# patrickzbhe/ray-tracing-series-rust

Measured on AMD Instinct MI355X. Metric: Msamples/s (pixels x spp) on Book-1 final scene, higher is better.
Workload: dtype f64

## Files before the change

ray-tracing-series-rust_amd/csrc/core/integrator.hpp:

```cpp
#pragma once
#include "shading.hpp"

namespace rt {

struct PathState {
  Ray ray;
  Color product;
  Color output;
  int32_t depth;
  Rng rng;
};

RT_HD void path_begin(const RenderParams& rp, uint32_t i, uint32_t j, uint32_t sample, PathState* ps) {
  uint64_t pixel_index = (uint64_t)j * (uint64_t)rp.image_width + (uint64_t)i;
  ps->rng = rng_for_sample(rp.seed, pixel_index, sample);
  real ru = rng_f64(ps->rng);
  real u = ((real)i + ru) / (real)(rp.image_width - 1);
  real rv = rng_f64(ps->rng);
  real v = ((real)j + rv) / (real)(rp.image_height - 1);
  ps->ray = camera_get_ray(rp.cam, u, v, ps->rng);
  ps->product = v3(1, 1, 1);
  ps->output = v3(0, 0, 0);
  ps->depth = rp.max_depth;
}

RT_HD bool path_bounce_begin(PathState* ps) {
  ps->depth -= 1;
#if defined(RT_F32)
  const real mag = rt_fabs(ps->ray.origin.x) + rt_fabs(ps->ray.origin.y) + rt_fabs(ps->ray.origin.z) +
                   rt_fabs(ps->ray.direction.x) + rt_fabs(ps->ray.direction.y) + rt_fabs(ps->ray.direction.z);
  if (!(mag < RT_INFINITY)) return true;
#endif
  return ps->depth < 0;
}

template <uint32_t F, bool COUNT>
RT_HD bool path_bounce_end(const SceneView& sv, const RenderParams& rp, PathState* ps, bool hit,
                           const HitRecord& rec, TraceCounters* cnt) {
  if (!hit) {
    ps->output += ps->product * rp.background;
    return true;
  }
  const FlatMaterial& m = sv.materials[rec.mat];
  Ray scattered;
  Color attenuation;
  bool did_scatter = material_scatter<F, COUNT>(sv, m, ps->ray, rec, ps->rng, &scattered, &attenuation, cnt);
  Color emitted = material_emitted<F, COUNT>(sv, m, rec, cnt);
  ps->output += emitted * ps->product;
  if (!did_scatter) return true;
  ps->product *= attenuation;
  ps->ray = scattered;
  return false;
}

enum LightKind : int32_t { LIGHT_RECT = 0, LIGHT_SPHERE = 1 };
struct FlatLight {
  int32_t kind;
  int32_t slot;
  int32_t prim;
  int32_t mat;
  real area;
  real cdf;
  real pmf;
};
struct LightView {
  const FlatLight* lights;
  const int32_t* slot_light;
  int32_t n_lights;
  int32_t pad;
};

#define RT_NEE_SHADOW_EPS real(1e-6)

RT_HD real mis_power(real a, real b) {
  const real a2 = a * a, b2 = b * b;
  return a2 / (a2 + b2);
}

RT_HD real light_pdf_rect(const FlatRect& q, real area, Vec3 d) {
  const real dn = rt_fabs(q.axis == RECT_XY ? d.z : (q.axis == RECT_XZ ? d.y : d.x));
  const real d2 = length_squared(d);
  return d2 * rt_sqrt(d2) / (dn * area);
}
RT_HD real sphere_cone_one_minus(const FlatSphere& s, Point3 p) {
  const Vec3 oc = v3(s.cx, s.cy, s.cz) - p;
  const real d2 = length_squared(oc), r2 = s.radius * s.radius;
  if (!(d2 > r2)) return real(0.0);
  const real k = r2 / d2;
  return k / (real(1.0) + rt_sqrt(real(1.0) - k));
}
RT_HD real light_pdf_sphere(const FlatSphere& s, Point3 p) {
  const real om = sphere_cone_one_minus(s, p);
  return om > real(0.0) ? real(1.0) / (real(2.0) * RT_PI * om) : real(0.0);
}
RT_HD real light_pdf(const SceneView& sv, const LightView& lv, int32_t k, Point3 p, Point3 q) {
  const FlatLight& L = lv.lights[k];
  const real ps = L.kind == LIGHT_RECT ? light_pdf_rect(sv.rects[L.prim], L.area, q - p) : light_pdf_sphere(sv.spheres[L.prim], p);
  return L.pmf * ps;
}

RT_HD real nee_bsdf_pdf(int32_t kind, const HitRecord& rec, Vec3 dir) {
  if (kind == MAT_ISOTROPIC) return real(1.0) / (real(4.0) * RT_PI);
  const real c = dot(rec.normal, dir) / length(dir);
  return c > real(0.0) ? c / RT_PI : real(0.0);
}

template <uint32_t F, bool COUNT, class STACK>
RT_HD Color nee_connect(const SceneView& sv, const LightView& lv, const PathState* ps, const HitRecord& rec, int32_t kind,
                        Color albedo, Rng& rng, STACK& stack, TraceCounters* cnt) {
  const real ul = rng_f64(rng);
  int32_t k = 0;
  while (k + 1 < lv.n_lights && !(ul < lv.lights[k].cdf)) ++k;
  const FlatLight& L = lv.lights[k];
  const real u1 = rng_f64(rng), u2 = rng_f64(rng);
  const Point3 p = rec.p;
  Point3 q;
  real pdf_sa;
  HitRecord lrec;
  lrec.u = real(0.0); lrec.v = real(0.0);
  if (L.kind == LIGHT_RECT) {
    const FlatRect& r = sv.rects[L.prim];
    const real a = r.a0 + u1 * (r.a1 - r.a0), b = r.b0 + u2 * (r.b1 - r.b0);
    q = r.axis == RECT_XY ? v3(a, b, r.k) : (r.axis == RECT_XZ ? v3(a, r.k, b) : v3(r.k, a, b));
    if (F & F_IMAGE) {
      lrec.u = (a - r.a0) / (r.a1 - r.a0);
      lrec.v = (b - r.b0) / (r.b1 - r.b0);
    }
    pdf_sa = light_pdf_rect(r, L.area, q - p);
  } else {
    const FlatSphere& s = sv.spheres[L.prim];
    const Point3 c = v3(s.cx, s.cy, s.cz);
    const real om = sphere_cone_one_minus(s, p);
    if (!(om > real(0.0))) return v3(0, 0, 0);
    const Vec3 w = unit(c - p);
    const Vec3 a = rt_fabs(w.x) > real(0.9) ? v3(0, 1, 0) : v3(1, 0, 0);
// ... 113 lines not shown
```

ray-tracing-series-rust_amd/csrc/hip/render.hip:

```cpp
#include <hip/hip_runtime.h>
#include <cstdio>
#include <cstdlib>
#include <algorithm>
#include <chrono>
#include <cfloat>
#include <cmath>
#include <cstring>
#include <new>
#include <type_traits>
#include <utility>
#include <string>
#include <vector>
#include "../../../include/rtx_abi.h"
#include "../core/cull32.hpp"
#include "../core/integrator.hpp"
#include "../host/flat_scene.hpp"
#include "../host/light_table.hpp"
#include "device_buffer.hpp"
#include "f32_bridge.hpp"
#ifndef RTX_F32_TU
#include "abi_internal.hpp"
#else
namespace rtx { void set_error(const std::string& msg); }
#endif

namespace rtx {

#include "pass_items.inc"

struct FlatNode4;
typedef const FlatNode4 FlatNode4Dev;
struct WorldDesc;

struct LdsSceneDims {
  uint32_t n_nodes, n_refs, n_spheres, n_moving;
  uint32_t node_dwords;
  uint32_t n_uni;
};

struct VoteTop {
  int32_t n;
  int32_t all_rects;
  int32_t k[8];
  uint32_t ref[8];
  rt::FlatRect rect[8];
};

enum class ForcedKernel { none, simple, vote, world, wavefront };

struct TraceSwitches {
  ForcedKernel kernel = ForcedKernel::none;
  bool diag = false;
  int ring = -1, wide = -1, scene_lds = -1;
  bool vote_top = true, tri_direct = true, mat_lds = true, perlin_lds = true;
  bool mv_common = true, motion = true, motion_axis = true;
  bool single_leaf = true, pass_pipeline = true, validate = false;
  uint32_t chunk = TRACE_CHUNK;
  uint32_t world_threshold = 8;
  uint32_t walk_threshold = 0, regen_min = 0, leaf_weight = 0;
  uint32_t wf_paths = 1u << 22, wf_refill = 16, wf_check = 8;
  int wf_occ = 4;
  bool wf_verbose = false;
};

struct Workspace {
  DeviceBuffer<double> samples;
  DeviceBuffer<double> accum;
  DeviceBuffer<rt::TraceCounters> counters;
  DeviceBuffer<unsigned int> work_counter;
  DeviceBuffer<unsigned long long> diag;
  hipEvent_t ev[2] = {nullptr, nullptr};
  hipStream_t aux_stream = nullptr;
  hipEvent_t ev_pass[3] = {nullptr, nullptr, nullptr};
  DeviceBuffer<unsigned char> wave_mem;
  uint32_t* wave_host_ctrl = nullptr;
};

struct VotePlan {
  bool ok = false;
  int32_t bvh_pos = 0;
  int32_t tri_base = -1;
  VoteTop top;
  int blocks_per_cu[2] = {1, 1};
  bool ring[2] = {false, false};
  uint32_t tables = 0;
  size_t tables_bytes = 0;
};

struct WidePlan {
  FlatNode4Dev* nodes4 = nullptr;
  int levels = 0;
  int vote_blocks_per_cu = 1;
};

struct WorldPlan {
  const WorldDesc* desc = nullptr;
  uint32_t mat_lds = 0, tex_lds = 0;
  uint32_t perlin_lds = 0;
  int blocks_per_cu[5][2] = {{1, 1}, {1, 1}, {1, 1}, {1, 1}, {1, 1}};
};

struct LdsFit {
  bool ok = false;
  uint32_t ring_cap = 0;
  uint32_t levels = 0;
  LdsSceneDims dims = {0, 0, 0, 0, 0, 0};
};

struct LdsPlan {
  LdsFit plain;
  LdsFit motion;
  int motion_axis = -1;
  double motion_t0 = 0.0, motion_t1 = 0.0;
  bool mv_common = false;
  double mv_t0 = 0.0, mv_t1 = 1.0;
};

struct WalkTuning {
  uint32_t walk_threshold = 18;
  uint32_t regen_min = 1;
  uint32_t leaf_weight = 3;
  bool single_leaf = false;
};

struct DeviceScene {
  int device = -1;
  std::vector<DeviceBuffer<void>> allocations;
  rt::SceneView view;
  size_t scene_bytes = 0;
  int n_cu = 256;
  double gravity_time_limit = 1e300;
  TraceSwitches sw;
  Workspace ws;
  VotePlan vote;
  WidePlan wide;
  WorldPlan world;
  LdsPlan lds;
  WalkTuning walk;
  rt::LightView lights = {nullptr, nullptr, 0, 0};
};

#define HIP_TRY(expr)                                                                      \
  do {                                                                                     \
    hipError_t _e = (expr);                                                                \
    if (_e != hipSuccess) {                                                                \
      set_error(std::string(#expr) + ": " + hipGetErrorString(_e));                        \
      return RTX_EHIP;                                                                     \
    }                                                                                      \
  } while (0)

template <class T>
static rtx_status upload_array(DeviceScene* ds, const std::vector<T>& v, const T** out) {
  *out = nullptr;
  if (v.empty()) return RTX_OK;
  DeviceBuffer<void> b;
  size_t bytes = v.size() * sizeof(T);
  HIP_TRY(b.alloc(bytes));
  HIP_TRY(hipMemcpy(b, v.data(), bytes, hipMemcpyHostToDevice));
  ds->scene_bytes += bytes;
  *out = (const T*)(void*)b;
  ds->allocations.push_back(std::move(b));
  return RTX_OK;
}

static void free_device_scene(DeviceScene* ds) {
  if (!ds) return;
  Workspace& ws = ds->ws;
  if (ws.wave_host_ctrl) (void)hipHostFree(ws.wave_host_ctrl);
  for (int i = 0; i < 2; ++i)
    if (ws.ev[i]) (void)hipEventDestroy(ws.ev[i]);
  for (int i = 0; i < 3; ++i)
    if (ws.ev_pass[i]) (void)hipEventDestroy(ws.ev_pass[i]);
  if (ws.aux_stream) (void)hipStreamDestroy(ws.aux_stream);
  delete ds;
}

template <class T>
__device__ __forceinline__ T dev_load_uniform(const T* p) { return *(const __attribute__((address_space(4))) T*)(p); }

__device__ __forceinline__ unsigned long long wave_ballot(bool p) { return __builtin_amdgcn_ballot_w64(p); }

#define TRACE_BLOCK 256
struct LdsStack {
  int32_t* base;
  int n;
  static constexpr bool kBottom = false;
  __device__ __forceinline__ void reset() { n = 0; }
  __device__ __forceinline__ void push(int32_t v) { base[n * TRACE_BLOCK] = v; ++n; }
  __device__ __forceinline__ int32_t pop() { --n; return base[n * TRACE_BLOCK]; }
  __device__ __forceinline__ bool empty() const { return n == 0; }
};
struct LdsStackB {
  int32_t* base;
  int n;
  static constexpr bool kBottom = true;
  __device__ __forceinline__ void reset() { base[0] = 0x7fffffff; n = 1; }
  __device__ __forceinline__ void init() { reset(); }
  __device__ __forceinline__ void push(int32_t v) { base[n * TRACE_BLOCK] = v; ++n; }
  __device__ __forceinline__ int32_t pop() { --n; return base[n * TRACE_BLOCK]; }
  __device__ __forceinline__ int32_t top() const { return base[(n - 1) * TRACE_BLOCK]; }
  __device__ __forceinline__ bool empty() const { return n <= 1; }
};

__device__ __forceinline__ void flush_counters(const rt::TraceCounters& c, rt::TraceCounters* g) {
  atomicAdd(&g->box_tests, c.box_tests);
  atomicAdd(&g->sphere_tests, c.sphere_tests);
  atomicAdd(&g->moving_sphere_tests, c.moving_sphere_tests);
  atomicAdd(&g->rect_tests, c.rect_tests);
  atomicAdd(&g->triangle_tests, c.triangle_tests);
  atomicAdd(&g->scatters, c.scatters);
  atomicAdd(&g->texels, c.texels);
  atomicAdd(&g->perlin_calls, c.perlin_calls);
  atomicAdd(&g->rays, c.rays);
  atomicAdd(&g->samples, c.samples);
}

#define DIAG_ADD(region, mask) do { if (DIAG) { dg[2 * (region)] += 1; dg[2 * (region) + 1] += (unsigned long long)__popcll(mask); } } while (0)
#include "trace_basic.inc"
#include "trace_vote.inc"
#include "trace_world.inc"
#include "trace_lds.inc"
#include "trace_wave.inc"
#include "post_kernels.inc"
#include "denoise.inc"
#ifndef RTX_F32_TU
#include "trace_nee.inc"
#endif

static int shard_row_count(int32_t height, const RtxShard& sh, int32_t row_limit) {
  int n = 0;
  for (int32_t j = 0; j < height && j < row_limit; ++j)
    if ((j / sh.block_rows) % sh.shard_count == sh.shard_index) ++n;
  return n;
}

static rtx_status validate(const void* s, const RtxCamera* cam, const RtxConfig* cfg,
                           const RtxShard* shard, RtxShard* sh_out) {
  if (!s || !cam || !cfg) { set_error("render: NULL scene, camera or config"); return RTX_EINVAL; }
  if (cfg->threads <= 0 || cfg->image_width <= 0 || cfg->samples_per_pixel <= 0 || cfg->max_depth <= 0) {
    set_error("render: Config::new asserts threads, image_width, samples_per_pixel, max_depth > 0 (world.rs:36-40)");
    return RTX_EINVAL;
  }
  if (rtx_image_height(cfg) <= 0) { set_error("render: image height <= 0 (Screen::new asserts, screen.rs:14)"); return RTX_EINVAL; }
  if (!(cam->time1 < cam->time2)) { set_error("render: camera time1 >= time2 (gen_range panics on an empty range, camera.rs:69)"); return RTX_EINVAL; }
  RtxShard sh = {0, 1, 1, 0};
  if (shard) sh = *shard;
  if (sh.shard_count <= 0 || sh.shard_index < 0 || sh.shard_index >= sh.shard_count || sh.block_rows <= 0) {
    set_error("render: bad shard");
    return RTX_EINVAL;
  }
  *sh_out = sh;
  return RTX_OK;
}

static rt::RenderParams make_params(const RtxCamera* cam, const RtxConfig* cfg) {
  rt::RenderParams rp;
  static_assert(sizeof(RtxCamera) == 24 * sizeof(double) && sizeof(rt::FlatCamera) == 24 * sizeof(rt::real), "camera layout");
  for (int k = 0; k < 24; ++k) ((rt::real*)&rp.cam)[k] = (rt::real)((const double*)cam)[k];
  rp.background = rt::v3(cfg->background[0], cfg->background[1], cfg->background[2]);
  rp.image_width = cfg->image_width;
  rp.image_height = rtx_image_height(cfg);
  rp.samples_per_pixel = cfg->samples_per_pixel;
  rp.max_depth = cfg->max_depth;
  rp.seed = cfg->seed;
  return rp;
}

static TraceSwitches read_switches() {
  auto num = [](const char* n, int lo, int hi, uint32_t dflt) { const char* s = getenv(n); return s && atoi(s) >= lo && atoi(s) <= hi ? (uint32_t)atoi(s) : dflt; };
  auto flag = [](const char* n) { const char* s = getenv(n); return s ? (atoi(s) != 0 ? 1 : 0) : -1; };
  TraceSwitches sw;
  if (const char* k = getenv("RTX_TRACE_KERNEL")) {
    const std::string s = k;
    if (s == "simple") sw.kernel = ForcedKernel::simple;
    else if (s == "vote" || s == "vote_diag") sw.kernel = ForcedKernel::vote;
    else if (s == "world" || s == "world_diag") sw.kernel = ForcedKernel::world;
    else if (s == "wavefront") sw.kernel = ForcedKernel::wavefront;
    sw.diag = s == "vote_diag" || s == "world_diag";
  }
  sw.ring = flag("RTX_RING"); sw.wide = flag("RTX_WIDE"); sw.scene_lds = flag("RTX_SCENE_LDS");
  sw.vote_top = flag("RTX_VOTE_TOP") != 0; sw.tri_direct = flag("RTX_TRI_DIRECT") != 0;
  sw.mat_lds = flag("RTX_MAT_LDS") != 0; sw.perlin_lds = flag("RTX_PERLIN_LDS") != 0;
  sw.mv_common = flag("RTX_MV_COMMON") != 0; sw.motion = flag("RTX_MOTION") != 0; sw.motion_axis = flag("RTX_MOTION_AXIS") != 0;
  sw.single_leaf = flag("RTX_SINGLE_LEAF") != 0; sw.pass_pipeline = flag("RTX_PASS_PIPELINE") != 0;
  sw.validate = getenv("RTX_VALIDATE") != nullptr;
  sw.chunk = num("RTX_CHUNK", 64, 65536, sw.chunk);
  sw.world_threshold = num("RTX_WORLD_THRESHOLD", 0, 64, sw.world_threshold);
  sw.walk_threshold = num("RTX_WALK_THRESHOLD", 1, 64, 0); sw.regen_min = num("RTX_REGEN_MIN", 1, 64, 0); sw.leaf_weight = num("RTX_LEAF_WEIGHT", 1, 64, 0);
  const char* wp = getenv("RTX_WF_PATHS");
  if (wp && atol(wp) >= 256 && atol(wp) <= (1l << 27)) sw.wf_paths = (uint32_t)atol(wp);
  sw.wf_refill = num("RTX_WF_REFILL", 1, 64, sw.wf_refill); sw.wf_check = num("RTX_WF_CHECK", 1, 4096, sw.wf_check);
  sw.wf_occ = (int)num("RTX_WF_OCC", 4, 6, (uint32_t)sw.wf_occ); sw.wf_verbose = getenv("RTX_WF_VERBOSE") != nullptr;
  return sw;
}

static size_t stack_bytes(uint32_t levels) { return (size_t)levels * TRACE_BLOCK * sizeof(int32_t); }

template <class K>
static int occupancy(K kernel, size_t lds) {
  int nb = 0;
  return hipOccupancyMaxActiveBlocksPerMultiprocessor(&nb, kernel, TRACE_BLOCK, lds) == hipSuccess ? nb : 0;
}

static uint32_t grid_size(uint32_t total, uint32_t block, uint64_t resident) {
  const uint64_t want = ((uint64_t)total + block - 1) / block;
  return (uint32_t)(want < resident ? want : resident);
}

struct PassArgs {
  rt::RenderParams rp;
  ShardMap sm;
  uint32_t s_begin, total, npix;
  double* samples;
  unsigned int* work_counter;
  hipStream_t stream;
  int preset;
  uint32_t feat;
  uint32_t stack_levels;
  size_t stack_lds;
  const uint32_t* active;
};

template <class Launch>
static void with_map(const PassArgs& a, Launch launch) {
  if (a.active) launch(ActiveMap{a.sm, a.active});
  else launch(a.sm);
}

template <class Launch>
static rtx_status run_diag(DeviceScene* ds, hipStream_t stream, Launch launch, const char* tag, int width, const char* const* names,
                           int n, unsigned long long (&h)[24]) {
  if (!ds->ws.diag) HIP_TRY(ds->ws.diag.alloc(sizeof(h)));
  HIP_TRY(hipMemsetAsync(ds->ws.diag, 0, sizeof(h), stream));
  launch();
  HIP_TRY(hipStreamSynchronize(stream));
  HIP_TRY(hipMemcpy(h, ds->ws.diag, sizeof(h), hipMemcpyDeviceToHost));
  for (int k = 0; k < n; ++k)
    fprintf(stderr, "[%s] %-*s executions %llu lanes %llu mean lanes %.2f\n", tag, width, names[k], h[2 * k], h[2 * k + 1],
            h[2 * k] ? (double)h[2 * k + 1] / (double)h[2 * k] : 0.0);
  return RTX_OK;
}

struct LeafScan { uint32_t max_count = 0, max_end = 0; };
static LeafScan scan_leaves(const FlatScene& fs) {
  LeafScan s;
  for (const rt::FlatNode& nd : fs.nodes)
    for (int ch = 0; ch < 2; ++ch)
      if (nd.child[ch] < 0) {
        s.max_count = std::max(s.max_count, rt::leaf_count(nd.child[ch]));
        s.max_end = std::max(s.max_end, rt::leaf_first(nd.child[ch]) + rt::leaf_count(nd.child[ch]));
      }
  return s;
}

static void plan_vote(DeviceScene* ds, const FlatScene& fs) {
  VotePlan& p = ds->vote;
  const TraceSwitches& sw = ds->sw;
  const size_t lds = stack_bytes((uint32_t)fs.max_stack + 1u), lds_ring = lds + (TRACE_BLOCK / 64) * ring_bytes(64);
  const bool ring_fits = lds_ring <= 64 * 1024;
  auto fit = [&](int preset, int nb0, int nb1, bool ring_by_default) {
    p.ring[preset] = ring_by_default && nb1 > 0 && nb1 >= nb0 && ring_fits;
    if (sw.ring >= 0 && nb1 > 0 && ring_fits) p.ring[preset] = sw.ring != 0;
    const int nb = p.ring[preset] ? nb1 : nb0;
    if (nb > 0) p.blocks_per_cu[preset] = nb;
  };
  fit(0, occupancy(k_trace_vote<P_SPHERES, false, false, false>, lds), occupancy(k_trace_vote<P_SPHERES, false, true, false>, lds_ring), true);
  fit(1, occupancy(k_trace_vote<P_MESH, false, false, false>, lds), occupancy(k_trace_vote<P_MESH, false, true, false>, lds_ring), false);

  memset(&p.top, 0, sizeof(p.top));
  p.top.n = -1;
  int n_bvh = 0, n_other = 0;
// ... 228 lines not shown

static void fit_lds(LdsFit* f, bool want_ring, uint32_t lds_max) {
  for (uint32_t cap : {64u, 48u, 0u})
    if ((want_ring || cap == 0u) && ldsk_layout(f->levels, cap, f->dims).total <= lds_max) {
      f->ok = true;
      f->ring_cap = cap;
      return;
    }
}

static rtx_status plan_lds(DeviceScene* ds, const FlatScene& fs, const LeafScan& leaves) {
  const bool single_bvh = fs.top_level.size() == 1 && fs.entries[fs.top_level[0]].kind == rt::ENTRY_BVH;
  if (!single_bvh || (fs.features & ~P_SPHERES) != 0 || fs.nodes32.size() > LDSK_MAX_NODES) return RTX_OK;
  LdsPlan& p = ds->lds;
  const TraceSwitches& sw = ds->sw;
  const uint32_t max_end = leaves.max_end, levels = (uint32_t)fs.max_stack + 1u;
  int lds_max = 0;
  (void)hipDeviceGetAttribute(&lds_max, hipDeviceAttributeMaxSharedMemoryPerBlock, ds->device);
  if (lds_max > 160 * 1024) lds_max = 160 * 1024;
  p.plain.levels = levels;
  p.plain.dims = {(uint32_t)fs.nodes32.size(), max_end, max_end, 0u, LDSK_NODE_DWORDS, 0u};
  if (!fs.moving_spheres.empty()) {
    bool same = sw.mv_common;
    for (const rt::FlatMovingSphere& ms : fs.moving_spheres)
      same = same && ms.time0 == fs.moving_spheres[0].time0 && ms.time1 == fs.moving_spheres[0].time1;
    if (same) { p.mv_common = true; p.mv_t0 = (double)fs.moving_spheres[0].time0; p.mv_t1 = (double)fs.moving_spheres[0].time1; }
  }
  if (fs.features & rt::F_MOVING_SPHERE) {
    p.plain.dims.n_uni = (uint32_t)fs.spheres.size();
    p.plain.dims.n_moving = max_end;
    p.plain.dims.n_spheres = 0u;
  }
  p.motion.levels = levels;
  p.motion.dims = p.plain.dims;
  p.motion.dims.node_dwords = LDSK_MOTION_NODE_DWORDS;
  {
    bool moves[3] = {false, false, false};
    for (const rt::FlatMotion32& m : fs.motion32)
      for (int ch = 0; ch < 2; ++ch)
        for (int a = 0; a < 3; ++a) moves[a] = moves[a] || m.dlo[ch][a] != 0.0f || m.dhi[ch][a] != 0.0f;
    if (!fs.motion32.empty() && moves[1] && !moves[0] && !moves[2] && sw.motion_axis) {
      p.motion_axis = 1;
      p.motion.dims.node_dwords = LDSK_MOTION1_NODE_DWORDS;
    }
  }
  if (leaves.max_count <= 4 && max_end <= LDSK_MAX_SLOTS && sw.scene_lds != 0 && lds_max > 0) {
    const bool want_ring = sw.ring != 0;
    fit_lds(&p.plain, want_ring, (uint32_t)lds_max);
    const rt::FlatEntry& be = fs.entries[fs.top_level[0]];
    if (p.plain.ok && !fs.motion32.empty() && (fs.features & rt::F_MOVING_SPHERE) && (double)be.f[0] < (double)be.f[1] && sw.motion) {
      p.motion_t0 = (double)be.f[0]; p.motion_t1 = (double)be.f[1];
      fit_lds(&p.motion, want_ring, (uint32_t)lds_max);
    }
  }
  if (p.plain.ok) {
    hipError_t ae = hipSuccess;
#define LDS_ATTR1(K) if (ae == hipSuccess) ae = hipFuncSetAttribute((const void*)K, hipFuncAttributeMaxDynamicSharedMemorySize, lds_max)
#define LDS_ATTR(FEAT, RINGF, MOTIONF) LDS_ATTR1((k_trace_lds<FEAT, RINGF, MOTIONF>)); LDS_ATTR1((k_trace_lds<FEAT, RINGF, MOTIONF, ActiveMap>))
    LDS_ATTR(P_SPHERES, true, 0u); LDS_ATTR(P_SPHERES, false, 0u); LDS_ATTR(P_STATIC_SPHERES, true, 0u); LDS_ATTR(P_STATIC_SPHERES, false, 0u);
    LDS_ATTR(P_SPHERES, true, 1u); LDS_ATTR(P_SPHERES, false, 1u); LDS_ATTR(P_SPHERES, true, 3u); LDS_ATTR(P_SPHERES, false, 3u);
#undef LDS_ATTR
#undef LDS_ATTR1
    if (ae != hipSuccess) { (void)hipGetLastError(); p.plain.ok = false; }
  }
  if (sw.scene_lds >= 0) {
    auto bytes = [](const LdsFit& f) { return f.ok ? ldsk_layout(f.levels, f.ring_cap, f.dims).total : 0u; };
    fprintf(stderr, "[rtx] RTX_SCENE_LDS: k_trace_lds %s (ring of %u, %u B of LDS); time-aware boxes %s (ring of %u, %u B)\n",
            p.plain.ok ? "on" : "off", p.plain.ring_cap, ldsk_layout(levels, p.plain.ring_cap, p.plain.dims).total,
            p.motion.ok ? "on" : "off", p.motion.ring_cap, bytes(p.motion));
  }
  return RTX_OK;
}

static rtx_status launch_lds(DeviceScene* ds, const PassArgs& a, const RtxCamera* cam) {
  const LdsPlan& p = ds->lds;
  HIP_TRY(hipMemsetAsync(a.work_counter, 0, sizeof(unsigned int), a.stream));
  const bool motion = p.motion.ok && (double)cam->time1 >= p.motion_t0 && (double)cam->time2 <= p.motion_t1;
  const LdsFit& f = motion ? p.motion : p.plain;
  const bool ring = f.ring_cap != 0u;
  const rt::real m_t0 = (rt::real)p.motion_t0, m_inv = (rt::real)(1.0 / (p.motion_t1 - p.motion_t0));
  const LdsKernelLayout L = ldsk_layout(f.levels, f.ring_cap, f.dims);
  const uint32_t grid = grid_size(a.total, LDSK_BLOCK, (uint64_t)ds->n_cu);
  const WalkTuning& wk = ds->walk;
#define LAUNCH_LDS2(FEAT, RINGF, MOTIONF)                                                                               \
  with_map(a, [&](auto map) {                                                                                           \
    hipLaunchKernelGGL(HIP_KERNEL_NAME(k_trace_lds<FEAT, RINGF, MOTIONF, decltype(map)>), dim3(grid), dim3(LDSK_BLOCK), L.total, \
                       a.stream, ds->view, a.rp, map, a.s_begin, a.total, a.npix, a.samples, a.work_counter, wk.leaf_weight, \
                       wk.walk_threshold | (wk.single_leaf ? 0x100u : 0u), ds->sw.chunk, f.ring_cap, f.levels, f.dims,  \
                       m_t0, m_inv, p.mv_common ? 1u : 0u, (rt::real)p.mv_t0, (rt::real)p.mv_t1);                        \
  })
#define LAUNCH_LDS(FEAT, MOTIONF) do { if (ring) { LAUNCH_LDS2(FEAT, true, MOTIONF); } else { LAUNCH_LDS2(FEAT, false, MOTIONF); } } while (0)
  if ((a.feat & ~P_STATIC_SPHERES) == 0) { LAUNCH_LDS(P_STATIC_SPHERES, 0u); }
  else if (motion && p.motion_axis == 1) { LAUNCH_LDS(P_SPHERES, 3u); }
  else if (motion) { LAUNCH_LDS(P_SPHERES, 1u); }
  else { LAUNCH_LDS(P_SPHERES, 0u); }
#undef LAUNCH_LDS
#undef LAUNCH_LDS2
  return RTX_OK;
}

template <bool COUNT>
static void launch_simple(const DeviceScene* ds, const PassArgs& a) {
  const uint32_t grid = grid_size(a.total, TRACE_BLOCK, (uint64_t)ds->n_cu * 8);
#define LAUNCH_SIMPLE2(FEAT, MAP)                                                                                       \
  hipLaunchKernelGGL(HIP_KERNEL_NAME(k_trace_simple<FEAT, COUNT, decltype(MAP)>), dim3(grid), dim3(TRACE_BLOCK), a.stack_lds, \
                     a.stream, ds->view, a.rp, MAP, a.s_begin, a.total, a.npix, a.samples, ds->ws.counters)
#define LAUNCH_SIMPLE(FEAT) with_map(a, [&](auto map) { LAUNCH_SIMPLE2(FEAT, map); })
  const bool inst = (a.feat & rt::F_INSTANCE) != 0;
  if constexpr (COUNT) {
    if (inst) { LAUNCH_SIMPLE2(P_INST, a.sm); } else { LAUNCH_SIMPLE2(P_ALL, a.sm); }
  } else {
    if (a.preset == 0) { LAUNCH_SIMPLE(P_SPHERES); }
    else if (a.preset == 1) { LAUNCH_SIMPLE(P_MESH); }
    else if (inst) { LAUNCH_SIMPLE(P_INST); }
    else { LAUNCH_SIMPLE(P_ALL); }
  }
#undef LAUNCH_SIMPLE
#undef LAUNCH_SIMPLE2
}

#ifndef RTX_F32_TU
static rtx_status launch_nee(const DeviceScene* ds, const PassArgs& a) {
  HIP_TRY(hipMemsetAsync(a.work_counter, 0, sizeof(unsigned int), a.stream));
  const int preset = (a.feat & rt::F_INSTANCE) ? 3 : ((a.feat & ~P_MESH_ROOM) == 0 ? 0 : ((a.feat & rt::F_GRAVITY_SPHERE) ? 2 : 1));
#define LAUNCH_NEE(FEAT, MAP)                                                                                                   \
  do {                                                                                                                          \
    const int nb = occupancy(k_trace_nee<FEAT, decltype(MAP)>, a.stack_lds);                                                    \
    const uint32_t grid = grid_size(a.total, TRACE_CHUNK, (uint64_t)ds->n_cu * (uint64_t)(nb > 0 ? nb : 1) * (TRACE_BLOCK / 64)); \
    hipLaunchKernelGGL(HIP_KERNEL_NAME(k_trace_nee<FEAT, decltype(MAP)>), dim3((grid + TRACE_BLOCK / 64 - 1) / (TRACE_BLOCK / 64)),     \
                       dim3(TRACE_BLOCK), a.stack_lds, a.stream, ds->view, ds->lights, a.rp, MAP, a.s_begin, a.total, a.npix,     \
                       a.samples, a.work_counter);                                                                              \
  } while (0)
  with_map(a, [&](auto map) {
    if (preset == 0) LAUNCH_NEE(P_MESH_ROOM, map);
    else if (preset == 1) LAUNCH_NEE(P_ANY, map);
    else if (preset == 3) LAUNCH_NEE(P_INST, map);
    else LAUNCH_NEE(P_ALL, map);
  });
#undef LAUNCH_NEE
  return RTX_OK;
}
#endif

static rtx_status wave_pass(DeviceScene* ds, const PassArgs& a) {
  Workspace& ws = ds->ws;
  const hipStream_t stream = a.stream;
  uint32_t P = ds->sw.wf_paths;
  if ((uint64_t)P > (uint64_t)a.total) P = a.total;
  P = (P + WF_SEG - 1u) & ~(WF_SEG - 1u);
  const uint32_t n_seg = P / WF_SEG;
  const size_t R = sizeof(rt::real);
  const size_t bytes = 64 + (size_t)P * (16 + 7 * R + 3 * R + 3 * R + R + 4 + 4 + 4 + 4) + (size_t)n_seg * 8;
  HIP_TRY(ws.wave_mem.grow(bytes, stream));
  if (!ws.wave_host_ctrl) HIP_TRY(hipHostMalloc((void**)&ws.wave_host_ctrl, 4 * sizeof(uint32_t), hipHostMallocDefault));
  WavePool pool;
  {
    unsigned char* m = ws.wave_mem;
    pool.ctrl = (uint32_t*)m; m += 64;
    pool.rng = (unsigned long long*)m; m += (size_t)P * 16;
    pool.ray = (rt::real*)m; m += (size_t)P * 7 * R;
    pool.product = (rt::real*)m; m += (size_t)P * 3 * R;
    pool.output = (rt::real*)m; m += (size_t)P * 3 * R;
    pool.hit_t = (rt::real*)m; m += (size_t)P * R;
    pool.depth = (int32_t*)m; m += (size_t)P * 4;
    pool.g = (uint32_t*)m; m += (size_t)P * 4;
    pool.hit_ref = (uint32_t*)m; m += (size_t)P * 4;
    pool.free_list = (uint32_t*)m; m += (size_t)P * 4;
    pool.n_free = (uint32_t*)m; m += (size_t)n_seg * 4;
    pool.cursor = (uint32_t*)m; m += (size_t)n_seg * 4;
    pool.P = P;
  }
  const int preset = a.preset;
  const bool wide = preset == 1 && ds->wide.nodes4 != nullptr;
  const uint32_t levels = wide ? (uint32_t)ds->wide.levels : a.stack_levels;
  const size_t lds = stack_bytes(levels);
  if (lds > 64 * 1024) { set_error("render: BVH too deep for the LDS traversal stack"); return RTX_EUNSUPPORTED; }
  const bool room = (a.feat & ~P_MESH_ROOM) == 0;
  const int occ = ds->sw.wf_occ;
  const uint32_t leaf_weight = ds->walk.leaf_weight, refill = ds->sw.wf_refill, bvh_pos = (uint32_t)ds->vote.bvh_pos;
#define WF_CASES(X)                                                                                                          \
  if (preset == 0) { X(P_SPHERES, false, 4); }                                                                               \
  else if (!wide) { X(P_MESH, false, 4); }                                                                                   \
  else if (room && occ == 5) { X(P_MESH_ROOM, true, 5); }                                                                    \
  else if (room && occ == 6) { X(P_MESH_ROOM, true, 6); }                                                                    \
  else if (room) { X(P_MESH_ROOM, true, 4); }                                                                                \
  else { X(P_MESH, true, 4); }
  int nb = 0;
  hipError_t oe = hipSuccess;
#define WF_OCC(FEAT, WIDEF, MB) oe = hipOccupancyMaxActiveBlocksPerMultiprocessor(&nb, k_wf_trace<FEAT, WIDEF, MB>, TRACE_BLOCK, lds)
  WF_CASES(WF_OCC)
#undef WF_OCC
  if (oe != hipSuccess || nb <= 0) { (void)hipGetLastError(); nb = 1; }
  const uint32_t tgrid = grid_size(P, TRACE_BLOCK, (uint64_t)ds->n_cu * (uint64_t)nb);
  hipLaunchKernelGGL(k_wf_init, dim3((P + 255u) / 256u), dim3(256), 0, stream, pool);
  uint32_t check_every = ds->sw.wf_check;
  int it = 0;
  for (;; ++it) {
    with_map(a, [&](auto map) {
      hipLaunchKernelGGL(HIP_KERNEL_NAME(k_wf_generate<decltype(map)>), dim3(n_seg), dim3(WF_SEG), 0, stream, pool, a.rp, map,
                         a.s_begin, a.total, a.npix);
    });
    if ((uint32_t)(it + 1) % check_every == 0u) {
      HIP_TRY(hipMemsetAsync(pool.ctrl, 0, 16, stream));
      hipLaunchKernelGGL(k_wf_count, dim3(256), dim3(256), 0, stream, pool);
      HIP_TRY(hipGetLastError());
      HIP_TRY(hipMemcpyAsync(ws.wave_host_ctrl, pool.ctrl, 4 * sizeof(uint32_t), hipMemcpyDeviceToHost, stream));
      HIP_TRY(hipStreamSynchronize(stream));
      if (ws.wave_host_ctrl[0] == 0u) break;
      if (ws.wave_host_ctrl[0] < P / 2u) check_every = 2;
      if (it > 100000000) { set_error("render: wavefront integrator did not converge"); return RTX_EHIP; }
    }
#define WF_LAUNCH(FEAT, WIDEF, MB)                                                                                           \
  do {                                                                                                                       \
    hipLaunchKernelGGL(HIP_KERNEL_NAME(k_wf_trace<FEAT, WIDEF, MB>), dim3(tgrid), dim3(TRACE_BLOCK), lds, stream, ds->view, pool, \
                       leaf_weight, refill, bvh_pos, ds->wide.nodes4, ds->vote.tri_base);                                    \
    hipLaunchKernelGGL(HIP_KERNEL_NAME(k_wf_shade<FEAT>), dim3(n_seg), dim3(WF_SEG), 0, stream, ds->view, pool, a.rp, a.samples, bvh_pos); \
  } while (0)
    WF_CASES(WF_LAUNCH)
#undef WF_LAUNCH
  }
#undef WF_CASES
  if (ds->sw.wf_verbose) fprintf(stderr, "[rtx] wavefront: %u slots, %d iterations, %d blocks per CU (%u stack levels)\n", P, it + 1, nb, levels);
  return RTX_OK;
}

static void plan_walk(DeviceScene* ds, const LeafScan& leaves) {
  WalkTuning& w = ds->walk;
  const TraceSwitches& sw = ds->sw;
  w.leaf_weight = leaves.max_count <= 1 ? 1u : 3u;
  w.single_leaf = leaves.max_count <= 1;
  if (ds->wide.nodes4) { w.leaf_weight = 1u; w.walk_threshold = 24u; w.regen_min = 8u; }
  else if (ds->lds.plain.ok) w.walk_threshold = 12u;
  if (sw.regen_min) w.regen_min = sw.regen_min;
  if (sw.leaf_weight) w.leaf_weight = sw.leaf_weight;
  if (!sw.single_leaf) w.single_leaf = false;
  if (sw.walk_threshold) w.walk_threshold = sw.walk_threshold;
}

static int32_t choose_trace_kernel(const DeviceScene* ds, int preset, bool count) {
  const ForcedKernel k = ds->sw.kernel;
  if (count || k == ForcedKernel::simple) return RTX_KERNEL_SIMPLE;
  if (ds->lds.plain.ok && preset == 0 && k == ForcedKernel::none) return RTX_KERNEL_LDS;
  if (ds->vote.ok && preset < 2 && k == ForcedKernel::wavefront) return RTX_KERNEL_WAVEFRONT;
  if (ds->vote.ok && preset < 2 && k != ForcedKernel::world) return RTX_KERNEL_VOTE;
  return RTX_KERNEL_WORLD;
}

typedef RtxSampleRange SampleRange;

struct PassPlan {
  uint32_t spp_pass;
  bool pipeline;
  size_t sample_bytes;
};

static rtx_status prepare_workspace(DeviceScene* ds, const RtxConfig* cfg, uint64_t npix, uint64_t npix_all, uint32_t spp, bool serial,
                                    hipStream_t stream, double** accum, PassPlan* pp) {
  Workspace& ws = ds->ws;
  uint64_t budget = cfg->sample_buffer_bytes;
  if (budget == 0) {
    budget = 24ull << 30;
    size_t free_b = 0, total_b = 0;
    if (hipMemGetInfo(&free_b, &total_b) == hipSuccess) {
      const uint64_t avail = ((uint64_t)free_b + ws.samples.bytes()) / 3;
      if (avail < budget) budget = avail;
    } else {
      (void)hipGetLastError();
    }
    if (budget < ws.samples.bytes()) budget = ws.samples.bytes();
  }
  const uint64_t per_sample_plane = npix * 24ull;
  uint32_t spp_pass = spp;
  const bool pipeline = ds->sw.pass_pipeline && !serial && ds->sw.kernel != ForcedKernel::simple && per_sample_plane > 0 &&
                        (uint64_t)spp * per_sample_plane > budget && budget / 2 >= per_sample_plane;
  const uint64_t pass_budget = pipeline ? budget / 2 : budget;
  if (per_sample_plane > 0 && (uint64_t)spp_pass * per_sample_plane > pass_budget) {
    spp_pass = (uint32_t)(pass_budget / per_sample_plane);
    if (spp_pass < 1) spp_pass = 1;
  }
  while (spp_pass > 1 && (uint64_t)spp_pass * npix >= 0xFFFF0000ull) --spp_pass;
  if ((uint64_t)spp_pass * npix >= 0xFFFF0000ull) { set_error("render: shard too large for one pass"); return RTX_EINVAL; }
  size_t need_samples = (size_t)spp_pass * per_sample_plane * (pipeline ? 2 : 1);
  if (need_samples > ws.samples.bytes()) {
    if (ws.samples) { HIP_TRY(hipStreamSynchronize(stream)); HIP_TRY(ws.samples.release()); }
    for (;;) {
      hipError_t me = ws.samples.alloc(need_samples);
      if (me == hipSuccess) break;
      (void)hipGetLastError();
      if (me != hipErrorOutOfMemory || spp_pass <= 1) {
        set_error(std::string("render: sample buffer of ") + std::to_string(need_samples) + " bytes: " + hipGetErrorString(me));
        return me == hipErrorOutOfMemory ? RTX_ENOMEM : RTX_EHIP;
      }
      spp_pass = (spp_pass + 1) / 2;
      need_samples = (size_t)spp_pass * per_sample_plane * (pipeline ? 2 : 1);
    }
  }
  if (!*accum) {
    HIP_TRY(ws.accum.grow((size_t)npix_all * 24, stream));
    *accum = ws.accum;
  }
  if (!ws.counters) HIP_TRY(ws.counters.alloc(sizeof(rt::TraceCounters)));
  if (!ws.work_counter) HIP_TRY(ws.work_counter.alloc(2 * sizeof(unsigned int)));
  if (pipeline && !ws.aux_stream) {
    HIP_TRY(hipStreamCreateWithFlags(&ws.aux_stream, hipStreamNonBlocking));
    for (int i = 0; i < 3; ++i) HIP_TRY(hipEventCreateWithFlags(&ws.ev_pass[i], hipEventDisableTiming));
  }
  if (!ws.ev[0]) { HIP_TRY(hipEventCreate(&ws.ev[0])); HIP_TRY(hipEventCreate(&ws.ev[1])); }
  *pp = {spp_pass, pipeline, need_samples};
  return RTX_OK;
}

template <bool COUNT>
static rtx_status render_impl(DeviceScene* ds, const RtxCamera* cam, const RtxConfig* cfg,
                              const RtxShard* shard, double* d_accum_out, uint8_t* d_rgb8_out,
                              hipStream_t stream, RtxRenderStats* stats, const SampleRange* range = nullptr) {
  RtxShard sh;
  rtx_status st = validate(ds, cam, cfg, shard, &sh);
  if (st != RTX_OK) return st;
  int cur = -1;
// ... 415 lines not shown
```

ray-tracing-series-rust_amd/csrc/hip/trace_lds.inc:

```

#define LDSK_BLOCK 1024
#define LDSK_DONE (-1)
#define LDSK_NO_REF 0xFFFFFFFFu
#define LDSK_MAX_SLOTS 8190u
#define LDSK_MAX_NODES 8191u
#define LDSK_NODE_DWORDS 21u
#ifndef LDSK_NODE_BURST
#define LDSK_NODE_BURST 1
#endif
#define LDSK_MOTION_NODE_DWORDS 39u
#define LDSK_MOTION1_NODE_DWORDS 27u

struct LdsKernelLayout {
  uint32_t off_ring, off_nodes, off_refs, off_spheres, off_moving, total;
};
__host__ __device__ inline LdsKernelLayout ldsk_layout(uint32_t levels, uint32_t ring_cap, const LdsSceneDims& d) {
  LdsKernelLayout L;
  uint32_t o = levels * LDSK_BLOCK * 2u;
  o = (o + 15u) & ~15u;
  L.off_ring = o; o += (LDSK_BLOCK / 64u) * ring_bytes(ring_cap);
  L.off_nodes = o; o += (d.n_nodes * d.node_dwords * 4u + 15u) & ~15u;
  L.off_refs = o;
  L.off_spheres = o; o += (d.n_spheres * (uint32_t)sizeof(rt::FlatSphere) + 15u) & ~15u;
  L.off_moving = o; o += (d.n_moving * (uint32_t)sizeof(rt::FlatMovingSphere) + 15u) & ~15u;
  L.total = o;
  return L;
}

struct LdsStack16 {
  unsigned short* base;
  int n;
  __device__ __forceinline__ void init() { base[0] = 0xFFFFu; n = 1; }
  __device__ __forceinline__ void reset() { n = 1; }
  __device__ __forceinline__ void push(int32_t v) { base[n * LDSK_BLOCK] = (unsigned short)v; ++n; }
  __device__ __forceinline__ int32_t pop() { --n; return (int32_t)(short)base[n * LDSK_BLOCK]; }
  __device__ __forceinline__ int32_t top() const { return (int32_t)(short)base[(n - 1) * LDSK_BLOCK]; }
};
__host__ __device__ __forceinline__ int32_t ldsk_item(int32_t child) {
  if (child >= 0) return child;
  return (int32_t)(short)(unsigned short)(0x8000u | (rt::leaf_first(child) << 2) | (rt::leaf_count(child) - 1u));
}

template <uint32_t F, bool RING, uint32_t MOTION, class SM = ShardMap>
__global__ __launch_bounds__(LDSK_BLOCK) void k_trace_lds(rt::SceneView sv, rt::RenderParams rp, SM sm,
                                                          uint32_t s_begin, uint32_t total, uint32_t npix,
                                                          double* __restrict__ samples, unsigned int* work_counter,
                                                          uint32_t leaf_weight, uint32_t walk_threshold, uint32_t chunk, uint32_t ring_cap,
                                                          uint32_t stack_levels, LdsSceneDims dims, rt::real motion_t0, rt::real motion_inv_dt,
                                                          uint32_t mv_common, rt::real mv_t0, rt::real mv_t1) {
  static_assert(!MOTION || (F & rt::F_MOVING_SPHERE), "time-aware boxes only make sense with moving spheres");
  const bool single_leaf = (walk_threshold & 0x100u) != 0u;
  walk_threshold &= 0xFFu;
  constexpr bool UNI = (F & rt::F_MOVING_SPHERE) != 0;
  constexpr uint32_t FL = UNI ? (F & ~rt::F_SPHERE) : F;
  static_assert(MOTION <= 4u, "0: no slopes, 1: all axes, 2 + a: axis a only");
  constexpr uint32_t ND = MOTION == 1u ? LDSK_MOTION_NODE_DWORDS : (MOTION >= 2u ? LDSK_MOTION1_NODE_DWORDS : LDSK_NODE_DWORDS);
  constexpr uint32_t CBD = MOTION == 1u ? 19u : (MOTION >= 2u ? 13u : 10u);
  constexpr uint32_t MA = MOTION >= 2u ? MOTION - 2u : 0u;
  constexpr uint32_t CB = CBD * 4u;
  constexpr uint32_t ITEM_OFF = CB - 4u;
  static_assert((F & ~(rt::F_SPHERE | rt::F_MOVING_SPHERE | rt::F_BVH | rt::F_LAMBERTIAN | rt::F_METAL |
                       rt::F_DIELECTRIC | rt::F_CHECKER)) == 0, "k_trace_lds caches spheres and moving spheres only");
  extern __shared__ __attribute__((aligned(16))) unsigned char ldsk[];
  const LdsKernelLayout L = ldsk_layout(stack_levels, RING ? ring_cap : 0u, dims);
  const uint32_t lane = threadIdx.x & 63u;
  const rt::FlatEntry& bvh = sv.entries[sv.top_level[0]];
  const int32_t root = bvh.a | (sv.nodes32[bvh.a].axis << 13);
  const uint32_t first_ref = (uint32_t)bvh.b;

  uint32_t* const lds_nodes = (uint32_t*)(ldsk + L.off_nodes);
  rt::FlatSphere* const lds_spheres = (rt::FlatSphere*)(ldsk + L.off_spheres);
  rt::FlatMovingSphere* const lds_moving = (rt::FlatMovingSphere*)(ldsk + L.off_moving);
  {
    static_assert(sizeof(rt::FlatNode32) == 64 && offsetof(rt::FlatNode32, child) == 48 && offsetof(rt::FlatNode32, axis) == 56,
                  "the padded LDS copy assumes FlatNode32's layout");
    const uint32_t* src = (const uint32_t*)sv.nodes32;
    const uint32_t* msrc = (const uint32_t*)sv.motion32;
    for (uint32_t k = threadIdx.x; k < dims.n_nodes * 2u * CBD; k += LDSK_BLOCK) {
      const uint32_t node = k / (2u * CBD), field = k - node * (2u * CBD);
      const uint32_t c = field / CBD, r = field - c * CBD;
      uint32_t v;
      if (r < 9u) {
        const uint32_t a = r / 3u, t = r - a * 3u;
        v = MOTION ? msrc[node * 24u + (t == 1u ? 6u : 0u) + c * 3u + a]
                   : src[node * 16u + (t == 1u ? 6u : 0u) + c * 3u + a];
      } else if (MOTION == 1u && r < 18u) {
        const uint32_t a = (r - 9u) / 3u, t = (r - 9u) - a * 3u;
        v = msrc[node * 24u + (t == 1u ? 18u : 12u) + c * 3u + a];
      } else if (MOTION >= 2u && r < 12u) {
        const uint32_t t = r - 9u;
        v = msrc[node * 24u + (t == 1u ? 18u : 12u) + c * 3u + MA];
      } else {
        const int32_t child = (int32_t)src[node * 16u + 12u + c];
        int32_t item = ldsk_item(child);
        if (child >= 0) item |= sv.nodes32[child].axis << 13;
        v = (uint32_t)item;
      }
      lds_nodes[node * ND + field] = v;
    }
    if (UNI) {
      for (uint32_t k = threadIdx.x; k < dims.n_refs; k += LDSK_BLOCK) {
        const rt::PrimRef ref = sv.refs[first_ref + k];
        rt::FlatMovingSphere m;
        if (rt::primref_type(ref) == rt::PRIM_SPHERE) {
          const rt::FlatSphere sp = sv.spheres[rt::primref_index(ref)];
          m.c0[0] = sp.cx; m.c0[1] = sp.cy; m.c0[2] = sp.cz; m.c1[0] = sp.cx; m.c1[1] = sp.cy; m.c1[2] = sp.cz;
          m.time0 = rt::real(0.0); m.time1 = rt::real(1.0); m.radius = sp.radius; m.mat = sp.mat; m.pad = 0;
        } else {
          m = sv.moving_spheres[rt::primref_index(ref)];
        }
        lds_moving[k] = m;
      }
    } else {
      constexpr uint32_t SD = (uint32_t)(sizeof(rt::FlatSphere) / 4);
      uint32_t* ds = (uint32_t*)lds_spheres;
      const uint32_t* ss = (const uint32_t*)sv.spheres;
      for (uint32_t k = threadIdx.x; k < dims.n_refs * SD; k += LDSK_BLOCK) {
        const uint32_t slot = k / SD, field = k - slot * SD;
        ds[k] = ss[rt::primref_index(sv.refs[first_ref + slot]) * SD + field];
      }
    }
  }
  __syncthreads();
  rt::SceneView lsv = sv;
  lsv.spheres = lds_spheres;
  lsv.moving_spheres = lds_moving;

  LdsStack16 stack;
  stack.base = (unsigned short*)ldsk + threadIdx.x;
  stack.init();
  double* const ring_f = (double*)(ldsk + L.off_ring + (threadIdx.x >> 6) * ring_bytes(ring_cap));
  uint32_t* const ring_g = (uint32_t*)(ring_f + RING_F64 * ring_cap);
  uint32_t ring_n = 0;
  uint32_t chunk_pos = 0, chunk_end = 0;
  bool queue_empty = false;
  bool active = false;
  uint32_t g = 0;
  rt::PathState ps;
  bool midwalk = false;
  rt::Ray32 q = {0.f, 0.f, 0.f, 0.f, 0.f, 0.f, 0.f, 0.f};
  uint32_t dir_neg = 0;
  uint32_t off_x = 0, off_y = 12, off_z = 24;
  uint32_t flip_b = 0;
  float t_max32 = 0.f;
  float s32 = 0.f;
  rt::real mv_ratio = rt::real(0.0);
  int32_t cur = LDSK_DONE;
  rt::Closest best;
  best.t = 0.0; best.ref = LDSK_NO_REF; best.order = 0; best.hit = false;

  for (;;) {
    const unsigned long long need_mask = wave_ballot(!active);
    if (need_mask != 0ull) {
      const uint32_t n_need = (uint32_t)__popcll(need_mask);
      const uint32_t rank = lane_rank(need_mask);
      if (RING) {
#define RING_CAP ring_cap
#define RING_DIAG(mask)
#include "trace_ring.inc"
#undef RING_DIAG
#undef RING_CAP
      } else {
        if (chunk_pos >= chunk_end && !queue_empty) {
          uint32_t base = 0;
          if (lane == 0) base = atomicAdd(work_counter, chunk);
          base = __builtin_amdgcn_readfirstlane(base);
          if (base >= total) {
            queue_empty = true;
          } else {
            chunk_pos = base;
            chunk_end = (total - base < chunk) ? total : base + chunk;
          }
        }
        if (chunk_pos < chunk_end) {
          const uint32_t avail = chunk_end - chunk_pos;
          if (!active && rank < avail) {
            g = chunk_pos + rank;
            start_path(rp, sm, npix, s_begin, g, &ps);
            active = true;
          }
          chunk_pos += (n_need < avail) ? n_need : avail;
        }
      }
    }
    if (wave_ballot(active) == 0ull) break;
    if (active && !midwalk) {
      if (rt::path_bounce_begin(&ps)) {
        store_sample(samples, g, ps.output);
        active = false;
      } else {
        q = rt::make_ray32(ps.ray, rt::ray_t_min(ps.ray));
        dir_neg = rt::ray_dir_neg(ps.ray);
        off_x = (dir_neg & 1u) << 2; off_y = 12u + ((dir_neg & 2u) << 1); off_z = 24u + (dir_neg & 4u);
        flip_b = ((dir_neg & 1u) * CB) | (((dir_neg >> 1) & 1u) * (CB << 8)) | (((dir_neg >> 2) & 1u) * (CB << 16));
        t_max32 = __builtin_huge_valf();
        if (UNI && mv_common != 0u) mv_ratio = (ps.ray.time - mv_t0) / (mv_t1 - mv_t0);
        if (MOTION) s32 = __builtin_fminf(__builtin_fmaxf((float)((ps.ray.time - motion_t0) * motion_inv_dt), 0.f), 1.f);
        best.t = RT_INFINITY; best.ref = LDSK_NO_REF; best.order = 0;
        stack.reset();
        cur = root;
        midwalk = true;
      }
    }
    const uint32_t threshold = (queue_empty && ring_n == 0u) ? 1u : walk_threshold;
    auto node_step = [&]() {
      const unsigned char* nd = (const unsigned char*)(lds_nodes + ((uint32_t)cur & 0x1FFFu) * ND);
      const uint32_t first_b = __builtin_amdgcn_ubfe(flip_b, ((uint32_t)cur >> 10) & 0x18u, 8u);
      const unsigned char* bf = nd + first_b;
      const unsigned char* bs = nd + (CB - first_b);
      const float *fx = (const float*)(bf + off_x), *fy = (const float*)(bf + off_y), *fz = (const float*)(bf + off_z);
      const float *sx = (const float*)(bs + off_x), *sy = (const float*)(bs + off_y), *sz = (const float*)(bs + off_z);
      const int32_t top = stack.top();
      bool hf, hs;
      if (MOTION >= 2u) {
        constexpr uint32_t SO = 9u - 3u * MA;
        const float* fm = MA == 0u ? fx : (MA == 1u ? fy : fz);
        const float* sm = MA == 0u ? sx : (MA == 1u ? sy : sz);
        const float fn = __builtin_fmaf(s32, fm[SO], fm[0]), ff = __builtin_fmaf(s32, fm[SO + 1u], fm[1]);
        const float sn = __builtin_fmaf(s32, sm[SO], sm[0]), sf = __builtin_fmaf(s32, sm[SO + 1u], sm[1]);
        hf = rt::cull32_may_hit_nf_pos(MA == 0u ? fn : fx[0], MA == 0u ? ff : fx[1], MA == 1u ? fn : fy[0], MA == 1u ? ff : fy[1],
                                       MA == 2u ? fn : fz[0], MA == 2u ? ff : fz[1], q, t_max32);
        hs = rt::cull32_may_hit_nf_pos(MA == 0u ? sn : sx[0], MA == 0u ? sf : sx[1], MA == 1u ? sn : sy[0], MA == 1u ? sf : sy[1],
                                       MA == 2u ? sn : sz[0], MA == 2u ? sf : sz[1], q, t_max32);
      } else if (MOTION) {
        hf = rt::cull32_may_hit_nf_pos(__builtin_fmaf(s32, fx[9], fx[0]), __builtin_fmaf(s32, fx[10], fx[1]), __builtin_fmaf(s32, fy[9], fy[0]),
                                   __builtin_fmaf(s32, fy[10], fy[1]), __builtin_fmaf(s32, fz[9], fz[0]), __builtin_fmaf(s32, fz[10], fz[1]), q, t_max32);
        hs = rt::cull32_may_hit_nf_pos(__builtin_fmaf(s32, sx[9], sx[0]), __builtin_fmaf(s32, sx[10], sx[1]), __builtin_fmaf(s32, sy[9], sy[0]),
                                   __builtin_fmaf(s32, sy[10], sy[1]), __builtin_fmaf(s32, sz[9], sz[0]), __builtin_fmaf(s32, sz[10], sz[1]), q, t_max32);
      } else {
        hf = rt::cull32_may_hit_nf_pos(fx[0], fx[1], fy[0], fy[1], fz[0], fz[1], q, t_max32);
        hs = rt::cull32_may_hit_nf_pos(sx[0], sx[1], sy[0], sy[1], sz[0], sz[1], q, t_max32);
      }
      const int32_t cf = *(const int32_t*)(bf + ITEM_OFF), cs = *(const int32_t*)(bs + ITEM_OFF);
      const bool both = hf && hs;
      if (both) stack.base[stack.n * LDSK_BLOCK] = (unsigned short)cs;
      cur = hf ? cf : (hs ? cs : top);
      stack.n += (int)both - (int)!(hf || hs);
    };
    auto leaf_test = [&](uint32_t slot) {
      const rt::PrimRef ref = rt::make_primref(UNI ? rt::PRIM_MOVING_SPHERE : rt::PRIM_SPHERE, slot);
      rt::real t;
      bool ok;
      if (UNI && mv_common != 0u) {
        const rt::FlatMovingSphere& sp = lds_moving[slot];
        const rt::Point3 c0 = rt::load_v3(sp.c0), c1 = rt::load_v3(sp.c1);
        ok = rt::sphere_root(c0 + mv_ratio * (c1 - c0), sp.radius, ps.ray, rt::ray_t_min(ps.ray), best.t, &t);
      } else {
        ok = rt::prim_t<FL, false>(lsv, ref, ps.ray, rt::ray_t_min(ps.ray), best.t, &t, nullptr);
      }
      if (ok && !(t == best.t && slot < best.order)) { best.t = t; best.ref = ref; best.order = slot; }
    };
    for (;;) {
      const bool is_node = cur >= 0;
      const bool is_leaf = cur < -1;
      const uint32_t n_node = (uint32_t)__popcll(wave_ballot(is_node)), n_leaf = (uint32_t)__popcll(wave_ballot(is_leaf));
      if (n_node + n_leaf < threshold) break;
      if (n_node * leaf_weight >= n_leaf) {
        if (is_node) node_step();
#if LDSK_NODE_BURST >= 2
        if (cur >= 0) node_step();
#endif
      } else {
        if (is_leaf) {
          const uint32_t f = ((uint32_t)cur & 0x7FFFu) >> 2;
          if (single_leaf) {
            leaf_test(f);
          } else {
            const uint32_t k = ((uint32_t)cur & 3u) + 1u;
            for (uint32_t i = 0; i < k; ++i) leaf_test(f + i);
          }
          t_max32 = rt::cull_round_up(best.t);
          cur = stack.pop();
        }
      }
    }
    if (midwalk && cur == LDSK_DONE) {
      midwalk = false;
      rt::HitRecord rec;
      const bool hit = best.ref != LDSK_NO_REF;
      if (hit) rt::prim_finalize<FL>(lsv, best.ref, ps.ray, best.t, &rec);
      if (rt::path_bounce_end<F, false>(sv, rp, &ps, hit, rec, nullptr)) {
        store_sample(samples, g, ps.output);
        active = false;
      }
    }
  }
}
```

Baseline: 7850.

## Batch rejection-sampled unit-sphere draws across the wave as a persistent state

Splits path shading into miss, draw and shade phases, and turns the rejection-sampling loop for random_in_unit_sphere into a wave-cooperative state (LDSK_DRAW). Lanes retry draws only while enough lanes need them, and the retries persist across outer iterations instead of serialising divergent rejection loops inside shading. A new draw_threshold tuning parameter is packed into the kernel argument. This removes divergence from the rejection loop, at the cost of extra state handling, a material lookup before shading, and sphere_sample possibly being lost or reset across iterations.

```diff
diff --git a/ray-tracing-series-rust_amd/csrc/core/integrator.hpp b/ray-tracing-series-rust_amd/csrc/core/integrator.hpp
--- a/ray-tracing-series-rust_amd/csrc/core/integrator.hpp
+++ b/ray-tracing-series-rust_amd/csrc/core/integrator.hpp
@@ -34,23 +34,35 @@
   return ps->depth < 0;
 }
 
+RT_HD void path_bounce_miss(const RenderParams& rp, PathState* ps) {
+  ps->output += ps->product * rp.background;
+}
+
 template <uint32_t F, bool COUNT>
-RT_HD bool path_bounce_end(const SceneView& sv, const RenderParams& rp, PathState* ps, bool hit,
-                           const HitRecord& rec, TraceCounters* cnt) {
-  if (!hit) {
-    ps->output += ps->product * rp.background;
-    return true;
-  }
-  const FlatMaterial& m = sv.materials[rec.mat];
+RT_HD bool path_bounce_scatter(const SceneView& sv, const FlatMaterial& m, PathState* ps, const HitRecord& rec,
+                               Vec3 sphere_sample, TraceCounters* cnt) {
   Ray scattered;
   Color attenuation;
-  bool did_scatter = material_scatter<F, COUNT>(sv, m, ps->ray, rec, ps->rng, &scattered, &attenuation, cnt);
+  bool did_scatter = material_scatter_with_sample<F, COUNT>(sv, m, ps->ray, rec, ps->rng, sphere_sample, &scattered, &attenuation, cnt);
   Color emitted = material_emitted<F, COUNT>(sv, m, rec, cnt);
   ps->output += emitted * ps->product;
   if (!did_scatter) return true;
   ps->product *= attenuation;
   ps->ray = scattered;
   return false;
+}
+
+template <uint32_t F, bool COUNT>
+RT_HD bool path_bounce_end(const SceneView& sv, const RenderParams& rp, PathState* ps, bool hit,
+                           const HitRecord& rec, TraceCounters* cnt) {
+  if (!hit) {
+    path_bounce_miss(rp, ps);
+    return true;
+  }
+  const FlatMaterial& m = sv.materials[rec.mat];
+  Vec3 sphere_sample = v3(0, 0, 0);
+  if (material_needs_sphere_sample(m.kind)) sphere_sample = random_in_unit_sphere(ps->rng);
+  return path_bounce_scatter<F, COUNT>(sv, m, ps, rec, sphere_sample, cnt);
 }
 
 enum LightKind : int32_t { LIGHT_RECT = 0, LIGHT_SPHERE = 1 };
diff --git a/ray-tracing-series-rust_amd/csrc/hip/render.hip b/ray-tracing-series-rust_amd/csrc/hip/render.hip
--- a/ray-tracing-series-rust_amd/csrc/hip/render.hip
+++ b/ray-tracing-series-rust_amd/csrc/hip/render.hip
@@ -58,6 +58,7 @@
   uint32_t chunk = TRACE_CHUNK;
   uint32_t world_threshold = 8;
   uint32_t walk_threshold = 0, regen_min = 0, leaf_weight = 0;
+  uint32_t draw_threshold = 0;
   uint32_t wf_paths = 1u << 22, wf_refill = 16, wf_check = 8;
   int wf_occ = 4;
   bool wf_verbose = false;
@@ -121,6 +122,7 @@
   uint32_t regen_min = 1;
   uint32_t leaf_weight = 3;
   bool single_leaf = false;
+  uint32_t draw_threshold = 8;
 };
 
 struct DeviceScene {
@@ -287,6 +289,7 @@
   sw.chunk = num("RTX_CHUNK", 64, 65536, sw.chunk);
   sw.world_threshold = num("RTX_WORLD_THRESHOLD", 0, 64, sw.world_threshold);
   sw.walk_threshold = num("RTX_WALK_THRESHOLD", 1, 64, 0); sw.regen_min = num("RTX_REGEN_MIN", 1, 64, 0); sw.leaf_weight = num("RTX_LEAF_WEIGHT", 1, 64, 0);
+  sw.draw_threshold = num("RTX_DRAW_THRESHOLD", 1, 64, 0);
   const char* wp = getenv("RTX_WF_PATHS");
   if (wp && atol(wp) >= 256 && atol(wp) <= (1l << 27)) sw.wf_paths = (uint32_t)atol(wp);
   sw.wf_refill = num("RTX_WF_REFILL", 1, 64, sw.wf_refill); sw.wf_check = num("RTX_WF_CHECK", 1, 4096, sw.wf_check);
@@ -681,11 +684,12 @@
   const LdsKernelLayout L = ldsk_layout(f.levels, f.ring_cap, f.dims);
   const uint32_t grid = grid_size(a.total, LDSK_BLOCK, (uint64_t)ds->n_cu);
   const WalkTuning& wk = ds->walk;
+  const uint32_t draw_threshold = std::max(1u, std::min(wk.draw_threshold, 65u - std::min(wk.walk_threshold, 64u)));
 #define LAUNCH_LDS2(FEAT, RINGF, MOTIONF)                                                                               \
   with_map(a, [&](auto map) {                                                                                           \
     hipLaunchKernelGGL(HIP_KERNEL_NAME(k_trace_lds<FEAT, RINGF, MOTIONF, decltype(map)>), dim3(grid), dim3(LDSK_BLOCK), L.total, \
                        a.stream, ds->view, a.rp, map, a.s_begin, a.total, a.npix, a.samples, a.work_counter, wk.leaf_weight, \
-                       wk.walk_threshold | (wk.single_leaf ? 0x100u : 0u), ds->sw.chunk, f.ring_cap, f.levels, f.dims,  \
+                       wk.walk_threshold | (wk.single_leaf ? 0x100u : 0u) | (draw_threshold << 16), ds->sw.chunk, f.ring_cap, f.levels, f.dims,  \
                        m_t0, m_inv, p.mv_common ? 1u : 0u, (rt::real)p.mv_t0, (rt::real)p.mv_t1);                        \
   })
 #define LAUNCH_LDS(FEAT, MOTIONF) do { if (ring) { LAUNCH_LDS2(FEAT, true, MOTIONF); } else { LAUNCH_LDS2(FEAT, false, MOTIONF); } } while (0)
@@ -834,6 +838,7 @@
   if (sw.leaf_weight) w.leaf_weight = sw.leaf_weight;
   if (!sw.single_leaf) w.single_leaf = false;
   if (sw.walk_threshold) w.walk_threshold = sw.walk_threshold;
+  if (sw.draw_threshold) w.draw_threshold = sw.draw_threshold;
 }
 
 static int32_t choose_trace_kernel(const DeviceScene* ds, int preset, bool count) {
diff --git a/ray-tracing-series-rust_amd/csrc/hip/trace_lds.inc b/ray-tracing-series-rust_amd/csrc/hip/trace_lds.inc
--- a/ray-tracing-series-rust_amd/csrc/hip/trace_lds.inc
+++ b/ray-tracing-series-rust_amd/csrc/hip/trace_lds.inc
@@ -1,6 +1,8 @@
 
 #define LDSK_BLOCK 1024
 #define LDSK_DONE (-1)
+#define LDSK_DRAW (-2)
+#define LDSK_SHADE (-3)
 #define LDSK_NO_REF 0xFFFFFFFFu
 #define LDSK_MAX_SLOTS 8190u
 #define LDSK_MAX_NODES 8191u
@@ -50,6 +52,7 @@
                                                           uint32_t mv_common, rt::real mv_t0, rt::real mv_t1) {
   static_assert(!MOTION || (F & rt::F_MOVING_SPHERE), "time-aware boxes only make sense with moving spheres");
   const bool single_leaf = (walk_threshold & 0x100u) != 0u;
+  const uint32_t draw_threshold = (walk_threshold >> 16) & 0xFFu;
   walk_threshold &= 0xFFu;
   constexpr bool UNI = (F & rt::F_MOVING_SPHERE) != 0;
   constexpr uint32_t FL = UNI ? (F & ~rt::F_SPHERE) : F;
@@ -137,7 +140,6 @@
   bool active = false;
   uint32_t g = 0;
   rt::PathState ps;
-  bool midwalk = false;
   rt::Ray32 q = {0.f, 0.f, 0.f, 0.f, 0.f, 0.f, 0.f, 0.f};
   uint32_t dir_neg = 0;
   uint32_t off_x = 0, off_y = 12, off_z = 24;
@@ -184,7 +186,7 @@
       }
     }
     if (wave_ballot(active) == 0ull) break;
-    if (active && !midwalk) {
+    if (active && cur == LDSK_DONE) {
       if (rt::path_bounce_begin(&ps)) {
         store_sample(samples, g, ps.output);
         active = false;
@@ -199,10 +201,10 @@
         best.t = RT_INFINITY; best.ref = LDSK_NO_REF; best.order = 0;
         stack.reset();
         cur = root;
-        midwalk = true;
-      }
-    }
-    const uint32_t threshold = (queue_empty && ring_n == 0u) ? 1u : walk_threshold;
+      }
+    }
+    const bool tail = queue_empty && ring_n == 0u;
+    const uint32_t threshold = tail ? 1u : walk_threshold;
     auto node_step = [&]() {
       const unsigned char* nd = (const unsigned char*)(lds_nodes + ((uint32_t)cur & 0x1FFFu) * ND);
       const uint32_t first_b = __builtin_amdgcn_ubfe(flip_b, ((uint32_t)cur >> 10) & 0x18u, 8u);
@@ -252,7 +254,7 @@
     };
     for (;;) {
       const bool is_node = cur >= 0;
-      const bool is_leaf = cur < -1;
+      const bool is_leaf = cur < -8;
       const uint32_t n_node = (uint32_t)__popcll(wave_ballot(is_node)), n_leaf = (uint32_t)__popcll(wave_ballot(is_leaf));
       if (n_node + n_leaf < threshold) break;
       if (n_node * leaf_weight >= n_leaf) {
@@ -274,14 +276,32 @@
         }
       }
     }
-    if (midwalk && cur == LDSK_DONE) {
-      midwalk = false;
-      rt::HitRecord rec;
-      const bool hit = best.ref != LDSK_NO_REF;
-      if (hit) rt::prim_finalize<FL>(lsv, best.ref, ps.ray, best.t, &rec);
-      if (rt::path_bounce_end<F, false>(sv, rp, &ps, hit, rec, nullptr)) {
+    if (active && cur == LDSK_DONE) {
+      if (best.ref == LDSK_NO_REF) {
+        rt::path_bounce_miss(rp, &ps);
         store_sample(samples, g, ps.output);
         active = false;
+      } else {
+        const int32_t mat = UNI ? lds_moving[best.order].mat : lds_spheres[best.order].mat;
+        cur = rt::material_needs_sphere_sample(sv.materials[mat].kind) ? LDSK_DRAW : LDSK_SHADE;
+      }
+    }
+    rt::Vec3 sphere_sample = rt::v3(0, 0, 0);
+    const uint32_t draw_min = tail ? 1u : draw_threshold;
+    for (;;) {
+      const bool is_draw = cur == LDSK_DRAW;
+      if ((uint32_t)__popcll(wave_ballot(is_draw)) < draw_min) break;
+      if (is_draw) {
+        if (rt::sphere_sample_try(ps.rng, &sphere_sample)) cur = LDSK_SHADE;
+      }
+    }
+    if (cur == LDSK_SHADE) {
+      cur = LDSK_DONE;
+      rt::HitRecord rec;
+      rt::prim_finalize<FL>(lsv, best.ref, ps.ray, best.t, &rec);
+      if (rt::path_bounce_scatter<F, false>(sv, sv.materials[rec.mat], &ps, rec, sphere_sample, nullptr)) {
+        store_sample(samples, g, ps.output);
+        active = false;
       }
     }
   }
```

Result: slower. 7722 (-1.6%).
